# stemangiola/ppcseq

Hardware: AMD Instinct MI355X
Metric: effective samples/sec (whole node) for NB hierarchical fit (higher is better)
Workload: dtype f64; 1 GPU; BASELINE cfg3: synthetic 20000 genes x 200 samples (seed 20253), C=2, K=1000; NUTS (Stan defaults) warm-up 150 + 250 kept draws/chain, 8 chains per GPU (cfg3 names 8 chains; chains are the sharded unit, so N GPUs run 8N chains); mode=chains, chains_total=8, lanes_per_gene=4, loglik_workgroups=939, ess_estimator=rank-normalised split-chain bulk-ESS, min over 6 hyper-parameters and lp__, grad_evals=1471121, divergent_after_warmup=0, round_structure=pipelined: merged log-likelihood / state-machine launch + gene kernel, stream_groups=library default (3 from eight chains on, 2 from four), rounds_last_step_all_groups=115040

## Files before the change

ppcseq_amd/build.py:

```python
from __future__ import annotations

import os
import subprocess
import sys
import threading

HERE = os.path.dirname(os.path.abspath(__file__))
CSRC = os.path.join(HERE, "csrc")
LIB = os.path.join(HERE, "libppcx.so")
TESTING_LIB = os.path.join(os.path.dirname(HERE), "tests", "libppcx_testing.so")
SOURCES = ["ppcx_kernels.hip", "ppcx_summary.hip", "ppcx_psis.hip", "ppcx_loo.hip", "ppcx_loo_predict.hip", "ppcx_reff.hip", "ppcx_ppc_exact.hip", "ppcx_ppc.hip",
           "ppcx_capi.hip", "ppcx_run.hip", "ppcx_fit_nuts.hip", "ppcx_fit_advi.hip", "ppcx_fit_api.hip"]
TESTING_SOURCES = ["ppcx_testing_math.hip"]
HEADERS = ["ppcx_math.h", "ppcx_disp.h", "ppcx_model.h", "ppcx_nuts.h", "ppcx_gene.h", "ppcx_kernels.h", "ppcx_summary.h", "ppcx_summary_dev.h", "ppcx_psis.h", "ppcx_psis_dev.h", "ppcx_loo.h", "ppcx_loo_ap.h", "ppcx_loo_dev.h", "ppcx_loo_predict.h", "ppcx_reff.h", "ppcx_nbcdf.h", "ppcx_ppc_exact.h", "ppcx_ppc.h", "ppcx_table.h", "ppcx_block.h", "ppcx_columns.h", "ppcx_host.h", "ppcx_testing.h",
           os.path.join("..", "..", "include", "ppcx.h")]


CODEGEN_FLAGS = ["-fno-slp-vectorize"]


def _sources(extra):
    return SOURCES + (TESTING_SOURCES if "-DPPCX_TESTING" in extra else [])


def _stale(lib: str, extra=()) -> bool:
    if not os.path.exists(lib):
        return True
    t = os.path.getmtime(lib)
    return any(os.path.getmtime(os.path.join(CSRC, f)) > t for f in _sources(extra) + HEADERS)


_COMPILERS = threading.BoundedSemaphore(16)


def _start_compiler(cmd):
    _COMPILERS.acquire()
    p = subprocess.Popen(cmd)
# ... 65 lines not shown
```

ppcseq_amd/csrc/ppcx_capi.hip:

```cpp
#include <math.h>
#include <stdlib.h>
#include <algorithm>
#include <memory>
#include "ppcx_host.h"

thread_local std::string g_err;
int fail(int code, const std::string& msg) { g_err = msg; return code; }
int hip_fail(hipError_t e, const char* what) { return fail(PPCX_ERR_HIP, std::string(what) + ": " + hipGetErrorString(e)); }
int hip_done(const char* who, hipError_t e) {
  return e == hipSuccess ? PPCX_OK : who ? hip_fail(e, who) : fail(PPCX_ERR_HIP, hipGetErrorString(e));
}
#ifdef PPCX_TESTING
TestHooks g_test;
#endif

extern "C" int ppcx_version(void) { return PPCX_VERSION; }
extern "C" int ppcx_device_count(void) { int n = 0; if (hipGetDeviceCount(&n) != hipSuccess) return 0; return n; }
extern "C" const char* ppcx_last_error(void) { return g_err.c_str(); }
extern "C" int ppcx_device_memory(int device, unsigned long long* free_bytes, unsigned long long* total_bytes) {
  int ndev = 0;
  HIPCHK(hipGetDeviceCount(&ndev));
  if (device < 0 || device >= ndev) return fail(PPCX_ERR_ARG, "no such HIP device");
  HIPCHK(hipSetDevice(device));
  size_t f = 0, t = 0;
  HIPCHK(hipMemGetInfo(&f, &t));
  if (free_bytes) *free_bytes = (unsigned long long)f;
  if (total_bytes) *total_bytes = (unsigned long long)t;
  return PPCX_OK;
}

static double pass_cost(const ppcx_model* m, int L, int p, int n) {
  const int S = m->d.S;
  bool slope = false;
  for (int i = p; i < p + n; ++i) slope = slope || m->pos_slope[i];
  double slope_w = m->d.C > 2 ? 1.0 : 1.15;
#ifdef PPCX_TESTING
  if (g_test.slope_cost_permille > 0) slope_w = 1e-3 * g_test.slope_cost_permille;
#endif
  double lin_w = 2.5;
#ifdef PPCX_TESTING
  if (g_test.slope_cost_permille > 0) lin_w = 1e-3 * g_test.slope_cost_permille;
#endif
  const double sweep = (double)((S + L - 1) / L) * (!m->d.x0_is_one ? 2.5 : (slope && !m->d.x1_binary ? lin_w : (slope ? slope_w : 1.0)));
  return 5.8 + sweep;
}
static int resident_workgroups(const ppcx_model* m, int reserve) {
  int n = m->wgs_override > 0 ? m->wgs_override : m->n_cu * (reserve > 0 ? m->ls_wgs_per_cu : m->wgs_per_cu);
  n -= reserve;
  return n < 1 ? 1 : n;
}
constexpr double kTrimSlack = 0.0;
static int workgroups_per_chain(const ppcx_model* m, int L, int nch, int n_res, bool whole_runs = true, bool trim = false) {
  int nbpc = n_res / (nch < 1 ? 1 : nch);
  if (nbpc >= 8 && whole_runs) nbpc = nbpc / 8 * 8;
  if (nbpc < 1) nbpc = 1;
  const int gpw = 64 / L, npass = (m->d.G + gpw - 1) / gpw;
  if (nbpc > (npass + 3) / 4) nbpc = (npass + 3) / 4;
  if (trim) {
    double slack = kTrimSlack;
#ifdef PPCX_TESTING
    if (g_test.trim_slack_permille >= 0) slack = 1e-3 * g_test.trim_slack_permille;
#endif
    int maxp = (npass + 4 * nbpc - 1) / (4 * nbpc);
#ifdef PPCX_TESTING
    maxp += g_test.trim_extra_passes;
// ... 63 lines not shown
    const long pmax = ((long)(npass + wpc - 1) / wpc) * gpw;
    for (int j = 0; j < wpc; ++j) if (bounds[j + 1] - bounds[j] > pmax) bounds[j + 1] = (int)(bounds[j] + pmax);
    bounds[wpc] = G;
    for (int j = wpc - 1; j >= 0; --j) if (bounds[j + 1] - bounds[j] > pmax) bounds[j] = (int)(bounds[j + 1] - pmax);
  }
  DeviceBuffer<int> d_bounds;
  HIPCHK(d_bounds.alloc((size_t)(wpc + 1)));
  HIPCHK(hipMemcpy(d_bounds.p, bounds.data(), sizeof(int) * (size_t)(wpc + 1), hipMemcpyHostToDevice));
  ppcx_model::Plan& pl = m->plans[key];
  pl.nbpc = nbpc; std::swap(pl.d_bounds.p, d_bounds.p);
  *nbpc_out = pl.nbpc; *d_bounds_out = pl.d_bounds.p;
  return PPCX_OK;
}

static int upload_counts(ppcx_model* m, int n_excl, const int32_t* excl) {
  const int G = m->d.G, S = m->d.S, C = m->d.C;
  std::vector<int32_t> cnt(m->counts_host);
  for (int e = 0; e < n_excl; ++e) {
    if (excl[e] < 0 || excl[e] >= G * S) return fail(PPCX_ERR_ARG, "excluded cell id out of range");
    cnt[excl[e]] = -1;
  }
  std::vector<double> Sy(G, 0.0), SyE(G, 0.0), SyX((size_t)C * G, 0.0), SX((size_t)C * G, 0.0), ncell(G, 0.0), Lg1(G, 0.0);
  std::vector<unsigned char> gflags(G, 0);
  for (int g = 0; g < G; ++g) {
    double sy = 0, sye = 0, nc = 0, lg1 = 0;
    for (int s = 0; s < S; ++s) {
      const int y = cnt[(size_t)g * S + s];
      if (y < 0) { gflags[g] |= 1; continue; }
      sy += y; sye += (double)y * m->expo_host[s]; nc += 1.0; lg1 += lgamma((double)y + 1.0);
      for (int c = 0; c < C; ++c) { SyX[(size_t)c * G + g] += (double)y * m->X_host[(size_t)c * S + s]; SX[(size_t)c * G + g] += m->X_host[(size_t)c * S + s]; }
    }
    Sy[g] = sy; SyE[g] = sye; ncell[g] = nc; Lg1[g] = lg1;
  }
  HIPCHK(hipMemcpy(m->d_gflags.p, gflags.data(), (size_t)G, hipMemcpyHostToDevice));
  {
    std::vector<int> ord(G);
    for (int g = 0; g < G; ++g) ord[g] = g;
    const int K = m->d.K;
    std::stable_sort(ord.begin(), ord.end(), [&](int a, int b) {
      const bool sa = a < K && C >= 2, sb = b < K && C >= 2;
      if (sa != sb) return sa;
      return gflags[a] > gflags[b];
    });
    {
      int ns = 0;
      while (ns < G && ord[ns] < K && C >= 2) ++ns;
      constexpr int kOrderBlock = 16;
      const int nbs = (ns + kOrderBlock - 1) / kOrderBlock, nb = (G + kOrderBlock - 1) / kOrderBlock;
      const bool dear_slopes = m->d.x0_is_one && !m->d.x1_binary;
      if (ns > 0 && ns < G && nbs < nb && dear_slopes) {
        std::vector<int> mixed; mixed.reserve(G);
        int is = 0, ip = ns, sb = 0;
        for (int b = 0; b < nb; ++b) {
          const bool slope_block = sb < nbs && b == (int)((long long)sb * nb / nbs);
          if (slope_block && is < ns) { for (int k = 0; k < kOrderBlock && is < ns; ++k) mixed.push_back(ord[is++]); ++sb; }
          else { for (int k = 0; k < kOrderBlock && ip < G; ++k) mixed.push_back(ord[ip++]); }
        }
        while (is < ns) mixed.push_back(ord[is++]);
        while (ip < G) mixed.push_back(ord[ip++]);
        ord.swap(mixed);
      }
    }
    HIPCHK(hipMemcpy(m->d_order.p, ord.data(), sizeof(int) * (size_t)G, hipMemcpyHostToDevice));
    m->pos_slope.resize(G);
    for (int p = 0; p < G; ++p) m->pos_slope[p] = ord[p] < K && C >= 2;
    drop_plans(m);
  }
  HIPCHK(hipMemcpy(m->d_counts.p, cnt.data(), sizeof(int32_t) * cnt.size(), hipMemcpyHostToDevice));
  m->excluded_host.assign(cnt.size(), 0);
  for (size_t i = 0; i < cnt.size(); ++i) m->excluded_host[i] = cnt[i] < 0;
  {
    const hipError_t e = launch_disp_build_kernel(m->d_counts.p, G, S, nullptr, G, m->fit, m->d_disp.p, m->stream.s);
    if (e != hipSuccess) return fail(PPCX_ERR_HIP, std::string("dispersion-table kernel: ") + hipGetErrorString(e));
  }
  HIPCHK(hipMemcpy(m->d_Sy.p, Sy.data(), sizeof(double) * G, hipMemcpyHostToDevice));
  HIPCHK(hipMemcpy(m->d_SyE.p, SyE.data(), sizeof(double) * G, hipMemcpyHostToDevice));
  HIPCHK(hipMemcpy(m->d_SyX.p, SyX.data(), sizeof(double) * SyX.size(), hipMemcpyHostToDevice));
  HIPCHK(hipMemcpy(m->d_SX.p, SX.data(), sizeof(double) * SX.size(), hipMemcpyHostToDevice));
  HIPCHK(hipMemcpy(m->d_ncell.p, ncell.data(), sizeof(double) * G, hipMemcpyHostToDevice));
  HIPCHK(hipMemcpy(m->d_Lg1.p, Lg1.data(), sizeof(double) * G, hipMemcpyHostToDevice));
  HIPCHK(hipStreamSynchronize(m->stream.s));
  return PPCX_OK;
}

extern "C" int ppcx_model_create(int device, int G, int S, int C, int K, const int32_t* counts, const double* X,
                                 const double* exposure, double lambda_mu_mu, int n_excl, const int32_t* excl,
                                 ppcx_model** out) {
  if (!out) return fail(PPCX_ERR_ARG, "out is NULL");
  *out = nullptr;
  if (G < 1 || S < 1 || C < 1 || K < 0 || K > G) return fail(PPCX_ERR_ARG, "need G>=1, S>=1, C>=1, 0<=K<=G");
  if (C > kMaxC) return fail(PPCX_ERR_LIMIT, "C exceeds the 16 design columns this build supports");
  if ((long long)G * S > 2000000000LL) return fail(PPCX_ERR_LIMIT, "G*S exceeds int32 cell ids");
  if (!counts || !X || !exposure || (n_excl > 0 && !excl)) return fail(PPCX_ERR_ARG, "NULL input buffer");
  for (long long i = 0; i < (long long)G * S; ++i) if (counts[i] < 0) return fail(PPCX_ERR_ARG, "negative count");
  int ndev = 0;
  HIPCHK(hipGetDeviceCount(&ndev));
  if (device < 0 || device >= ndev) return fail(PPCX_ERR_ARG, "no such HIP device");
// ... 25 lines not shown
    return fail(PPCX_ERR_LIMIT, "more than 8 design columns are supported for designs of a column of ones and 0 / 1 indicator columns only");
  if (const char* e = getenv("PPCX_PIPELINE")) if (atoi(e) == 0) m->opt_pipelined = 0;
  if (const char* e = getenv("PPCX_STREAM_GROUPS")) { const int v = atoi(e); if (v >= 1) m->opt_stream_groups = v; }
  if (loglik_lds_bytes(m->d) > 160u * 1024u)
    return fail(PPCX_ERR_LIMIT, "the per-sample constants (S * C doubles; S * (2 + C) for a design without a column of ones) do not fit the 160 KB of LDS of a compute unit beside the 20 KB of tables");
  m->wgs_per_cu = loglik_resident_workgroups_per_cu(m->CM, m->d);
  if (m->wgs_per_cu < 1) return fail(PPCX_ERR_LIMIT, "the log-likelihood kernel cannot be resident with S * (2 + C) doubles of per-sample constants in LDS");
  m->ls_wgs_per_cu = ls_resident_workgroups_per_cu(m->CM, m->d);
  std::vector<double> E(S);
  for (int s = 0; s < S; ++s) E[s] = exp(exposure[s]);
  HIPCHK(m->stream.create());
  HIPCHK(m->d_counts.alloc(((size_t)G * S + 512)));
  HIPCHK(hipMemset(m->d_counts.p, 0, sizeof(int32_t) * ((size_t)G * S + 512)));
  HIPCHK(m->d_E.alloc(S));
  HIPCHK(m->d_expo.alloc(S));
  HIPCHK(m->d_X.alloc((size_t)S * C));
  HIPCHK(m->d_Sy.alloc(G));
  HIPCHK(m->d_SyE.alloc(G));
  HIPCHK(m->d_SyX.alloc((size_t)C * G));
  HIPCHK(m->d_SX.alloc((size_t)C * G));
  HIPCHK(m->d_ncell.alloc(G));
  HIPCHK(m->d_disp.alloc((size_t)G * kDispGeneDoubles));
  HIPCHK(m->d_gflags.alloc((size_t)G));
  disp_fit_init(m->fit);
  HIPCHK(m->d_Lg1.alloc(G));
  HIPCHK(m->d_logtab.alloc(2 * kLogTabSize));
  { double tab[2 * kLogTabSize]; fill_log_table(tab); HIPCHK(hipMemcpy(m->d_logtab.p, tab, sizeof(tab), hipMemcpyHostToDevice)); }
  HIPCHK(m->d_wintab.alloc(2 * kWinTabSize));
  { std::vector<double> wt(2 * kWinTabSize); fill_window_log_table(wt.data()); HIPCHK(hipMemcpy(m->d_wintab.p, wt.data(), sizeof(double) * wt.size(), hipMemcpyHostToDevice)); }
  m->e_min = m->e_max = E[0];
  for (int s = 1; s < S; ++s) { if (E[s] < m->e_min) m->e_min = E[s]; if (E[s] > m->e_max) m->e_max = E[s]; }
  HIPCHK(m->d_order.alloc((size_t)G));
  HIPCHK(hipMemcpy(m->d_E.p, E.data(), sizeof(double) * S, hipMemcpyHostToDevice));
  HIPCHK(hipMemcpy(m->d_expo.p, exposure, sizeof(double) * S, hipMemcpyHostToDevice));
  HIPCHK(hipMemcpy(m->d_X.p, X, sizeof(double) * (size_t)S * C, hipMemcpyHostToDevice));
  const int rc = upload_counts(m, n_excl, excl);
  if (rc != PPCX_OK) return rc;
  choose_launch(m, 1);
  *out = owner.release();
  return PPCX_OK;
}
extern "C" int ppcx_model_create_shard_strided(int device, int G_total, int S, int C, int K_total, int g0, int gene_stride, int n_genes,
                                               const int32_t* counts_shard, const double* X, const double* exposure,
                                               double lambda_mu_mu, int n_excl, const int32_t* excl_local, ppcx_model** out) {
  if (g0 < 0 || gene_stride < 1 || n_genes < 1 || K_total < 0 || K_total > G_total ||
      (long long)g0 + (long long)gene_stride * (n_genes - 1) >= G_total) return fail(PPCX_ERR_ARG, "bad gene shard");
// ... 108 lines not shown
```

ppcseq_amd/csrc/ppcx_gene.h:

```cpp
#pragma once
#include "ppcx_nuts.h"


namespace ppcx {

template <int CM>
struct GeneCtx {
  static constexpr int NCM = CM + 1;
  int gg, ncoord;
  bool active, has_slopes, fast, two;
  int idx[NCM];
  double q[NCM];
  GeneParams<CM> gp;
};

PPCX_HD void coord_consts(const Dims& d, const VecRef& v, int i, double q) {
  if (i >= d.off_sigma_raw && i < d.off_tail) {
    v.at(V_C0, i) = fast_exp(-q); v.at(V_C2, i) = q;
  } else if (i >= d.off_intercept && i < d.off_sigma_raw) {
    v.at(V_C0, i) = fast_exp(q);
    if (d.raw_consts) v.at(V_C2, i) = q;
  }
}

// ... 17 lines not shown
  x.gp.coef[0] = x.q[0];
#pragma unroll
  for (int cc = 1; cc < CM; ++cc) x.gp.coef[cc] = (x.has_slopes && cc < d.C) ? x.q[cc + 1] : 0.0;
  x.gp.sigma_raw = x.q[1];
  x.gp.phi = x.active ? v.at(V_C0, x.idx[1]) : 1.0;
  x.gp.invphi = 0.0;
}
template <int CM>
PPCX_HD void gene_load(const Dims& d, const Cmd& c, const VecRef& v, int g, GeneCtx<CM>& x) {
  constexpr int NCM = CM + 1;
  gene_index<CM>(d, g, x);
#pragma unroll
  for (int j = 0; j < NCM; ++j) x.q[j] = j < x.ncoord ? v.at(V_Q0 + 3 * c.dir, x.idx[j]) : 0.0;
  gene_params<CM>(d, v, x);
}

struct CellData {
  const int* counts;
  const double* disp;
  const unsigned char* gflags;
  const double* Sy;
  const double* ncell;
  double e_min, e_max;
};

struct GenePre { double phi, sigma, a0, Sy, n; int flags; };
PPCX_HD GenePre gene_pre_load(const Dims& d, const VecRef& v, const CellData& m, int g) {
  GenePre r;
  r.phi = v.at(V_C0, d.off_sigma_raw + g);
  r.sigma = v.at(V_C2, d.off_sigma_raw + g);
  r.a0 = v.at(V_C0, d.off_intercept + g);
  r.Sy = m.Sy[g]; r.n = m.ncell[g]; r.flags = m.gflags[g];
  return r;
}
template <int L> struct DispDeal {
  static constexpr int NL = L >= 8 ? 4 : (L >= 4 ? 2 : 1);
  static constexpr int CH = kDispStride / NL;
};

template <int CM, int L, int MODE, bool MASKED, bool WIN>
PPCX_HD void sweep_cells(int S, const int* row, const double* sE, const double* sX1, int sub, double A, double A1, double one,
                         const GeneParams<CM>& gp, const double* tab, CellAcc<CM>& acc, const double* ec = nullptr, int C = 2) {
  const int nmin = S / L;
  const int nlane = nmin + (sub < S - nmin * L ? 1 : 0);
  const int* p = row + sub;
  const double* q = sE + sub;
  const double* qx = sX1 + sub;
  int y0 = p[0], y1 = p[L], y2 = p[2 * L], y3 = p[3 * L];
  int k = 0;
#define PPCX_SWEEP_CELL(Y, E, XB, OFF, COND)                                                    \
  if ((COND) && (!MASKED || (Y) >= 0)) {                                                        \
    if (MODE == 1) { const double a1_ = (XB) != 0.0 ? A1 : A;                                   \
                     const double rho_ = WIN ? cell_eval_win<CM, true>(Y, E, a1_, one, gp, tab, acc) : cell_eval<CM, true>(Y, E, a1_, gp, tab, acc); \
                     acc.Tx[1] = fma(XB, rho_, acc.Tx[1]); }                                    \
    else if (MODE == 2) {                                                                       \
      double a_ = (XB) != 0.0 ? A1 : A; double xk_[CM];                                         \
      _Pragma("unroll") for (int cc = 2; cc < CM; ++cc) { xk_[cc] = cc < C ? qx[(cc - 1) * S + (OFF)] : 0.0; a_ = xk_[cc] != 0.0 ? a_ * ec[cc] : a_; } \
      const double rho_ = WIN ? cell_eval_win<CM, true>(Y, E, a_, one, gp, tab, acc) : cell_eval<CM, true>(Y, E, a_, gp, tab, acc); \
      acc.Tx[1] = fma(XB, rho_, acc.Tx[1]);                                                     \
      _Pragma("unroll") for (int cc = 2; cc < CM; ++cc) acc.Tx[cc] = fma(xk_[cc], rho_, acc.Tx[cc]); \
// ... 100 lines not shown
  const double sigma = pre.sigma;
  gp.sigma_raw = sigma;
  gp.invphi = fast_rcp(gp.phi);
  const double A = pre.a0 * gp.invphi;
  const bool masked = (pre.flags & 1) != 0;
  const int* row = m.counts + (long)g * S;
  constexpr int NL = DispDeal<L>::NL, CH = DispDeal<L>::CH;
  const DispRef dr = disp_ref(sigma);
  const int fn = L == 1 ? 0 : sub / NL, jch = L == 1 ? 0 : sub - fn * NL;
  const bool tab_lane = dr.in && (L == 1 || fn < 2);
  const double* pc = m.disp + (((long)g * kDispPanels + dr.panel) * 2 + (fn & 1)) * kDispStride + jch * CH;
  double cf[CH], cf2[L == 1 ? CH : 1];
#pragma unroll
  for (int k = 0; k < CH; ++k) cf[k] = 0.0;
  cf2[0] = 0.0;
  if (tab_lane) {
#pragma unroll
    for (int k = 0; k < CH; ++k) cf[k] = pc[k];
    if (L == 1) {
#pragma unroll
      for (int k = 0; k < CH; ++k) cf2[k] = pc[kDispStride + k];
    }
  }
  CellAcc<CM> acc; acc.zero();
  PPCX_GSTAMP(5);
  if (GEN & 2) {
    if (PPCX_WAVE_ANY(generic)) {
      if (generic) generic_cells<CM, L>(d, c, v, g, has_slopes, row, sExpo, sX, sub, gp, tab, acc);
    }
  }
  GeneWindow gw; gw.k = 0; gw.ok = false; gw.scale = 1.0;
  bool win = false;
  if (!(GEN & 2) || PPCX_WAVE_ANY(!generic)) {
    if (!generic) {
      const bool any_masked = PPCX_WAVE_ANY(masked);
#define PPCX_SWEEP(MODE, A_LO, A_HI, A_, A1_, X1_, ...)                                                                  \
      gw = gene_window(fma(m.e_min, A_LO, 1.0), fma(m.e_max, A_HI, 1.0));                                                 \
      win = !any_masked && PPCX_WAVE_ALL(gw.ok);                                                                          \
      if (any_masked) sweep_cells<CM, L, MODE, true, false>(S, row, sE, X1_, sub, A_, A1_, 1.0, gp, tab, acc, ##__VA_ARGS__);   \
      else if (win) sweep_cells<CM, L, MODE, false, true>(S, row, sE, X1_, sub, (A_) * gw.scale, (A1_) * gw.scale, gw.scale, gp, wtab, acc, ##__VA_ARGS__); \
      else sweep_cells<CM, L, MODE, false, false>(S, row, sE, X1_, sub, A_, A1_, 1.0, gp, tab, acc, ##__VA_ARGS__);
      if ((GEN & 1) && PPCX_WAVE_ANY(lin)) {
        double be[CM];
        be[0] = 0.0;
#pragma unroll
        for (int cc = 1; cc < CM; ++cc) be[cc] = (lin && cc < d.C) ? v.at(V_C2, coef_index(d, cc, g)) : 0.0;
        if (any_masked) sweep_cells<CM, L, 3, true, false>(S, row, sE, sX + S, sub, A, A, 1.0, gp, tab, acc, be, d.C);
        else sweep_cells<CM, L, 3, false, false>(S, row, sE, sX + S, sub, A, A, 1.0, gp, tab, acc, be, d.C);
      } else if (CM > 2 && d.C > 2 && PPCX_WAVE_ANY(two)) {
        double ec[CM];
        ec[0] = 1.0;
        double a_lo = A, a_hi = A;
#pragma unroll
        for (int cc = 1; cc < CM; ++cc) {
          ec[cc] = (two && cc < d.C) ? v.at(V_C0, coef_index(d, cc, g)) : 1.0;
          a_lo = ec[cc] < 1.0 ? a_lo * ec[cc] : a_lo; a_hi = ec[cc] > 1.0 ? a_hi * ec[cc] : a_hi;
        }
        const double A1 = A * ec[1];
        PPCX_SWEEP(2, a_lo, a_hi, A, A1, sX + S, ec, d.C)
      } else if (PPCX_WAVE_ANY(two)) {
        const double A1 = two ? A * v.at(V_C0, coef_index(d, 1, g)) : A;
        PPCX_SWEEP(1, (A1 < A ? A1 : A), (A1 > A ? A1 : A), A, A1, sX + S)
      } else {
        PPCX_SWEEP(0, A, A, A, A, sX)
      }
#undef PPCX_SWEEP
    }
  }
  PPCX_GSTAMP(6);
  if (!win) gw.scale = 1.0;
  cell_acc_close<CM>(gp, acc, gw.scale, &o);
  if ((GEN & 1) && lin) o.Tx[0] = o.Sr;
  if (win && sub == 0 && gw.k != 0) {
    const double kd = (double)gw.k;
    const double klog2 = fma(kd, 6.93147180369123816490e-01, kd * 1.90821492927058770002e-10);
    o.lik -= klog2 * fma(gp.phi, pre.n, pre.Sy);
    o.dph -= klog2 * pre.n;
  }
  if (tab_lane) {
    double hv = cf[CH - 1];
#pragma unroll
    for (int k = CH - 2; k >= 0; --k) hv = fma(hv, dr.x, cf[k]);
    if (NL > 1) {
      const double x3 = dr.x * dr.x * dr.x, xc = CH == 3 ? x3 : x3 * x3;
      double xp = (jch & 1) ? xc : 1.0;
      if (NL > 2) xp = (jch & 2) ? xp * (xc * xc) : xp;
      hv *= xp;
    }
    if (L == 1) {
      double h2 = cf2[CH - 1];
#pragma unroll
      for (int k = CH - 2; k >= 0; --k) h2 = fma(h2, dr.x, cf2[k]);
      o.lik += hv; o.dph += h2;
    } else if (fn == 0) o.lik += hv;
    else o.dph += hv;
  }
  if (PPCX_WAVE_ANY(!dr.in)) {
    PPCX_KEEP_BRANCH();
    if (!dr.in) {
      double F, D;
      disp_row_at(row, S, sub, L, sigma, &F, &D);
      o.lik += F; o.dph += D;
    }
  }
}

struct GeneData { double Sy, SyE, ncell, Lg1, SyX[kMaxC], SX[kMaxC]; };
template <int CM>
PPCX_HD void gene_data_load(const Dims& d, int gg, const double* Sy, const double* SyE, const double* SyXg, const double* SXg,
                            const double* ncell, const double* Lg1, GeneData& o) {
  o.Sy = Sy[gg]; o.SyE = SyE[gg]; o.ncell = ncell[gg]; o.Lg1 = Lg1[gg];
#pragma unroll
  for (int cc = 0; cc < CM; ++cc) {
    if (cc == 0 && d.x0_is_one) { o.SyX[0] = o.Sy; o.SX[0] = o.ncell; continue; }
    o.SyX[cc] = (cc < d.C) ? SyXg[(long)cc * d.G + gg] : 0.0;
    o.SX[cc] = (cc < d.C) ? SXg[(long)cc * d.G + gg] : 0.0;
  }
}
// ... 221 lines not shown
```

ppcseq_amd/csrc/ppcx_host.h:

```cpp
#pragma once
#include <hip/hip_runtime.h>
#include <atomic>
#include <map>
#include <mutex>
#include <string>
#include <vector>
#include "../../include/ppcx.h"
#include "ppcx_kernels.h"
#include "ppcx_columns.h"

using namespace ppcx;

extern thread_local std::string g_err;
int fail(int code, const std::string& msg);
int hip_fail(hipError_t e, const char* what);
int hip_done(const char* who, hipError_t e);
#define HIPCHK(expr)                                                                       \
  do {                                                                                     \
    hipError_t e_ = (expr);                                                                \
    if (e_ != hipSuccess) return hip_fail(e_, #expr);                                      \
  } while (0)

#ifdef PPCX_TESTING
#include "ppcx_testing.h"
// ... 12 lines not shown
#endif

struct ppcx_model {
  int device;
  DeviceStream stream;
  Dims d;
  int CM, L = 64;
  int L_override = 0, wgs_override = 0;
  int n_cu = 256, wgs_per_cu = 4;
  int ls_wgs_per_cu = 0;
  int nblocks_chosen = 0;
  int opt_pipelined = -1, opt_stream_groups = 0;
  ppcx_progress_fn progress = nullptr; void* progress_user = nullptr; double progress_every = 1.0;
  std::vector<char> pos_slope;
  struct Plan { int nbpc = 0; DeviceBuffer<int> d_bounds; };
  std::map<std::pair<int, int>, Plan> plans;
  std::mutex plan_mutex;
  std::vector<int32_t> counts_host;
  std::vector<char> excluded_host;
  std::vector<double> X_host, expo_host;
  DeviceBuffer<int> d_counts;
  DeviceBuffer<double> d_E, d_expo, d_X, d_Sy, d_SyE, d_SyX, d_SX, d_ncell, d_Lg1;
  DeviceBuffer<double> d_disp;
  DeviceBuffer<unsigned char> d_gflags;
  DispFit fit;
  DeviceBuffer<double> d_logtab, d_wintab;
  double e_min = 1.0, e_max = 1.0;
  DeviceBuffer<int> d_order;
  int live_fits = 0;
  bool destroy_requested = false;
};

struct ppcx_fit {
  ppcx_model* m;
  NutsConfig cfg;
  int chains, n_keep, iter;
  DeviceBuffer<double> d_draws;
  DeviceBuffer<double> d_lp, d_stepsize, d_accept;
  DeviceBuffer<int> d_treedepth, d_nleap, d_div;
  double seconds = 0; long long grad_evals = 0;
  double kA_ms_mean = 0; long long kA_samples = 0; double kA_chain_launches_mean = 0;
  double kC_ms_mean = 0, kU_ms_mean = 0; long long launch_triples = 0;
  double advi_elbo = 0, advi_eta = 0; int advi_converged = 0;
  double ppc_ms = 0; long long ppc_draws = 0;
  long long xchg_ticks = 0, xchg_count = 0;
  std::vector<double> inv_metric;
// ... 46 lines not shown
```

ppcseq_amd/csrc/ppcx_kernels.h:

```cpp
#pragma once
#include <hip/hip_runtime.h>
#include "ppcx_gene.h"

namespace ppcx {

constexpr int kLdsPad = 256;
struct LoglikArgs {
  Dims d;
  CellData cd;
  const double* sampleE;
  const double* exposure;
  const double* X;
  double* vecs;
  long Dpad;
  const Cmd* cmds;
  double* sums;
  const double* logtab;
  const double* wintab;
  const int* order;
  int lgL;
  int nchains;
  const int* active;
  int nbpc;
  const int* bounds;
// ... 92 lines not shown
  const double* exposure; const double* X;
  double truncation_compensation, p_lo, p_hi;
  uint32_t k0;
  int n_gen, resample, n_cells;
  double* ci;
  int* counts_rng;
  int* scratch;
};

hipError_t launch_loglik_kernel(int CM, const LoglikArgs& a, hipStream_t st);
int loglik_resident_workgroups_per_cu(int CM, const Dims& d);
size_t loglik_lds_bytes(const Dims& d);
hipError_t launch_close_kernel(int CM, const CloseArgs& a, int nblocks, int nchains, hipStream_t st);
hipError_t launch_ls_kernel(int CM, const LoglikArgs& a, const StepArgs& sa, int n_srun, int n_chains_total, int spec, hipStream_t st,
                            hipEvent_t ev_start = nullptr, hipEvent_t ev_stop = nullptr);
int ls_resident_workgroups_per_cu(int CM, const Dims& d);
hipError_t launch_gene_kernel(int CM, const GeneArgs& a, int nblocks, int nchains, hipStream_t st);
hipError_t launch_step_kernel(const StepArgs& a, int nblocks, int nchains, hipStream_t st);
hipError_t launch_sum_shards_kernel(const ShardSumArgs& a, hipStream_t st);
hipError_t launch_update_kernel(const UpdateArgs& a, int nblocks, int nchains, hipStream_t st);
hipError_t launch_advi_kernel(const AdviArgs& a, int nblocks, hipStream_t st);
hipError_t launch_advi_elbo_kernel(const AdviElboArgs& a, hipStream_t st);
hipError_t launch_disp_build_kernel(const int* counts, int G, int S, const int* genes, int n_genes, const DispFit& fit, double* table, hipStream_t st);
hipError_t launch_gather_kernel(const double* draws, long n_rows, int D, const int* cols, int n_cols, double* out, hipStream_t st);
hipError_t launch_fill_kernel(double* p, long n, double val, hipStream_t st);

constexpr int kSummaryLdsDraws = 8192;
constexpr int kSummaryMaxChains = 128;
struct SummaryArgs {
  const double* x;
  int n_cols, M, n;
  int npad;
  double* out;
  double* scratch; long slice;
};
int summary_npad(int M, int n);
long summary_slice_doubles(int M, int n);
size_t summary_lds_bytes(int M, int n);
hipError_t launch_summary_gather_kernel(const double* draws, const double* lp, long rows, int D, const int* cols, int n_cols, double* out, hipStream_t st);
hipError_t launch_summary_kernel(const SummaryArgs& a, int nblocks, hipStream_t st);
constexpr size_t kSummaryScratchBytes = (size_t)256 << 20;
hipError_t summary_columns(const double* draws, const double* lp, int M, int n, int D, int n_cols, const int* cols, double* out,
                           size_t scratch_bytes, hipStream_t st);

constexpr int kPsisLdsDraws = 4096;
constexpr int kPsisMaxSel = 4096;
// ... 79 lines not shown
```

ppcseq_amd/csrc/ppcx_kernels.hip:

```cpp
#include <hip/hip_runtime.h>
#include <hip/hip_ext.h>
#include "ppcx_gene.h"
#include "ppcx_kernels.h"

namespace ppcx {

typedef int __attribute__((may_alias)) word_t;
typedef double2 __attribute__((may_alias)) dpair_t;

#ifndef PPCX_LOGLIK_OCC
#define PPCX_LOGLIK_OCC 2
#endif
#ifndef PPCX_LOGLIK_OCC_FAST
#define PPCX_LOGLIK_OCC_FAST 4
#endif
__device__ __forceinline__ double wave_xor_add_rt(double v, int lane_xor_mask) {
  const int src = (int)((threadIdx.x ^ (unsigned)lane_xor_mask) & 63u) << 2;
  const int lo = __builtin_amdgcn_ds_bpermute(src, __double2loint(v));
  const int hi = __builtin_amdgcn_ds_bpermute(src, __double2hiint(v));
  return v + __hiloint2double(hi, lo);
}
template <int CTRL, int ROW_MASK>
__device__ __forceinline__ double dpp_take(double v) {
  const int lo = __builtin_amdgcn_update_dpp(0, __double2loint(v), CTRL, ROW_MASK, 0xf, true);
// ... 884 lines not shown
  double* s_val = reinterpret_cast<double*>(s_row + ((S + 1) & ~1));
  for (int s = tid; s < S; s += kDispThreads) s_row[s] = counts[(long)g * S + s];
  __syncthreads();
  constexpr int NN = kDispPanels * kDispN;
  for (int t = tid; t < NN; t += kDispThreads) {
    const int p = t / kDispN, k = t - p * kDispN;
    double lo;
    const double sg = disp_node_sigma(fit, p, k, &lo);
    const DispPoint pt = disp_point(sg, lo);
    double F, D;
    disp_row(s_row, S, 0, 1, pt, &F, &D);
    s_val[(p * 2 + 0) * kDispN + k] = F; s_val[(p * 2 + 1) * kDispN + k] = D;
  }
  __syncthreads();
  for (int t = tid; t < 2 * kDispPanels; t += kDispThreads) {
    double out[kDispStride];
    disp_fit_panel(fit, s_val + t * kDispN, out);
    double* dst = table + (long)g * kDispGeneDoubles + (long)t * kDispStride;
#pragma unroll
    for (int m = 0; m < kDispStride; ++m) dst[m] = out[m];
  }
}

__global__ void ppcx_gather_kernel(const double* draws, long n_rows, int D, const int* cols, int n_cols, double* out) {
  const long i = (long)blockIdx.x * blockDim.x + threadIdx.x;
  if (i >= n_rows * n_cols) return;
  const long r = i / n_cols; const int cidx = (int)(i % n_cols);
  out[i] = draws[r * D + cols[cidx]];
}

__global__ void ppcx_xchg_abort_kernel(XchgArgs x) {
  const int k = threadIdx.x;
  if (k < x.nranks) sys_store(x.flags[k] + xchg_abort_index(x, x.rank), (unsigned long long)x.epoch);
  __threadfence_system();
}

__global__ void ppcx_fill_kernel(double* p, long n, double val) {
  const long i = (long)blockIdx.x * blockDim.x + threadIdx.x;
  if (i < n) p[i] = val;
}

static int loglik_generic_possible(const Dims& d) { return !d.x0_is_one ? 2 : ((d.C >= 2 && d.K > 0 && !d.x1_binary) ? 1 : 0); }
size_t loglik_lds_bytes(const Dims& d) {
  const size_t per_sample = loglik_generic_possible(d) == 2 ? (size_t)(2 + d.C) : (size_t)(d.C < 1 ? 1 : d.C);
  return sizeof(double) * (2 * kLogTabSize + 2 * kWinTabSize + (size_t)d.S * per_sample + 2 * kLdsPad);
}
// ... 85 lines not shown
}
hipError_t launch_update_kernel(const UpdateArgs& a, int nblocks, int nchains, hipStream_t st) {
  hipLaunchKernelGGL(ppcx_update_kernel, dim3(nblocks, nchains), dim3(256), 0, st, a);
  return hipGetLastError();
}
hipError_t launch_advi_kernel(const AdviArgs& a, int nblocks, hipStream_t st) {
  hipLaunchKernelGGL(ppcx_advi_kernel, dim3(nblocks), dim3(256), 0, st, a);
  return hipGetLastError();
}
hipError_t launch_advi_elbo_kernel(const AdviElboArgs& a, hipStream_t st) {
  hipLaunchKernelGGL(ppcx_advi_elbo_kernel, dim3(1), dim3(64), 0, st, a);
  return hipGetLastError();
}
size_t disp_build_lds_bytes(int S) { return sizeof(int) * (size_t)((S + 1) & ~1) + sizeof(double) * 2 * kDispPanels * kDispN; }
hipError_t launch_disp_build_kernel(const int* counts, int G, int S, const int* genes, int n_genes, const DispFit& fit, double* table, hipStream_t st) {
  const size_t lds = disp_build_lds_bytes(S);
  if (lds > 64u * 1024u) {
    hipError_t e = hipFuncSetAttribute((const void*)ppcx_disp_build_kernel, hipFuncAttributeMaxDynamicSharedMemorySize, (int)lds);
    if (e != hipSuccess) return e;
  }
  hipLaunchKernelGGL(ppcx_disp_build_kernel, dim3((unsigned)n_genes), dim3(kDispThreads), lds, st, counts, G, S, genes, n_genes, fit, table);
  return hipGetLastError();
}
hipError_t launch_gather_kernel(const double* draws, long n_rows, int D, const int* cols, int n_cols, double* out, hipStream_t st) {
  const long n = n_rows * n_cols;
  hipLaunchKernelGGL(ppcx_gather_kernel, dim3((unsigned)((n + 255) / 256)), dim3(256), 0, st, draws, n_rows, D, cols, n_cols, out);
  return hipGetLastError();
}
hipError_t launch_xchg_abort_kernel(const XchgArgs& x, hipStream_t st) {
  hipLaunchKernelGGL(ppcx_xchg_abort_kernel, dim3(1), dim3(64), 0, st, x);
  return hipGetLastError();
}
hipError_t launch_fill_kernel(double* p, long n, double val, hipStream_t st) {
  hipLaunchKernelGGL(ppcx_fill_kernel, dim3((unsigned)((n + 255) / 256)), dim3(256), 0, st, p, n, val);
  return hipGetLastError();
}

}
```

ppcseq_amd/csrc/ppcx_run.hip:

```cpp
#include <stdio.h>
#include <stdlib.h>
#include <string.h>
#include <chrono>
#include <dlfcn.h>
#include "ppcx_host.h"

#ifdef PPCX_TRACE
static unsigned long long* g_trace_dev = nullptr;
#endif
int work_alloc(Work& w, ppcx_model* m, int nchains) {
  const int D = m->d.D;
  if (!w.stream) w.stream = m->stream.s;
  w.Dpad = ((long)D + 31) / 32 * 32;
  w.nb_update = (D + 255) / 256;
  if (w.nb_update > 80) w.nb_update = 80;
  if (w.nb_update < 1) w.nb_update = 1;
  HIPCHK(w.vecs.alloc((size_t)nchains * V_COUNT * w.Dpad));
  w.nb_close = (m->d.G + 255) / 256;
  HIPCHK(w.partials.alloc((size_t)nchains * w.nb_close * PT_COUNT));
  HIPCHK(w.sums.alloc((size_t)nchains * (3 + m->CM) * m->d.G));
  HIPCHK(hipMemsetAsync(w.sums.p, 0, sizeof(double) * (size_t)nchains * (3 + m->CM) * m->d.G, w.stream));
  HIPCHK(w.done.alloc(nchains));
  HIPCHK(w.red.alloc((size_t)nchains * PT_COUNT));
  HIPCHK(hipMemsetAsync(w.red.p, 0, sizeof(double) * (size_t)nchains * PT_COUNT, w.stream));
// ... 43 lines not shown
}
int launch_step(ppcx_model* m, Work& w, int nchains, const RunIO& io, int phases, bool with_update) {
  StepArgs sa;
  step_args(m, w, io, phases, with_update, &sa);
  hipError_t e = launch_step_kernel(sa, w.nb_update, nchains, w.stream);
  if (e != hipSuccess) return fail(PPCX_ERR_HIP, std::string("step kernel: ") + hipGetErrorString(e));
  if (phases & STEP_ADVANCE) w.launches++;
  return PPCX_OK;
}
int launch_update(ppcx_model* m, Work& w, int nchains, const RunIO& io) {
  UpdateArgs ua;
  ua.d = m->d; ua.cmds = w.cmds[w.launches & 1].p; ua.vecs = w.vecs.p; ua.Dpad = w.Dpad;
  ua.draws = io.draws; ua.draws_chain_stride = io.draws_stride; ua.t0_out = w.t0[w.launches & 1].p;
  hipError_t e = launch_update_kernel(ua, w.nb_update, nchains, w.stream);
  if (e != hipSuccess) return fail(PPCX_ERR_HIP, std::string("update kernel: ") + hipGetErrorString(e));
  return PPCX_OK;
}
static int step_runs(int nchains, int nact) { return (nchains + nact - 1) / nact; }
static int loglik_args(ppcx_model* m, Work& w, int nchains, int reserve, LoglikArgs* out) {
  const int nact = w.n_active > 0 ? w.n_active : nchains;
  LoglikArgs& la = *out;
  int rc = plan_launch(m, nact, reserve, w.shared_chip, &la.nbpc, &la.bounds);
  if (rc != PPCX_OK) return rc;
  la.d = m->d; la.cd.counts = m->d_counts.p; la.cd.disp = m->d_disp.p; la.cd.gflags = m->d_gflags.p; la.cd.Sy = m->d_Sy.p; la.cd.ncell = m->d_ncell.p; la.cd.e_min = m->e_min; la.cd.e_max = m->e_max; la.sampleE = m->d_E.p; la.exposure = m->d_expo.p; la.X = m->d_X.p;
  la.vecs = w.vecs.p; la.Dpad = w.Dpad; la.cmds = w.cmds[w.launches & 1].p; la.sums = w.sums.p; la.logtab = m->d_logtab.p; la.wintab = m->d_wintab.p; la.order = m->d_order.p;
  la.lgL = 0; while ((1 << la.lgL) < m->L) ++la.lgL;
  la.nchains = nact; la.active = w.n_active > 0 ? w.active.p : nullptr;
#ifdef PPCX_TRACE
  la.trace = g_trace_dev;
#endif
  return PPCX_OK;
}
int launch_loglik(ppcx_model* m, Work& w, int nchains) {
  LoglikArgs la;
  int rc = loglik_args(m, w, nchains, 0, &la);
  if (rc != PPCX_OK) return rc;
  hipError_t e = launch_loglik_kernel(m->CM, la, w.stream);
  if (e != hipSuccess) return fail(PPCX_ERR_HIP, std::string("loglik kernel: ") + hipGetErrorString(e));
  return PPCX_OK;
}
static void close_args(ppcx_model* m, Work& w, CloseArgs* o) {
  CloseArgs& ca = *o;
  ca.d = m->d; ca.Sy = m->d_Sy.p; ca.SyE = m->d_SyE.p; ca.SyX = m->d_SyX.p; ca.SX = m->d_SX.p; ca.ncell = m->d_ncell.p; ca.Lg1 = m->d_Lg1.p;
  ca.sums = w.sums.p; ca.vecs = w.vecs.p; ca.Dpad = w.Dpad; ca.cmds = w.cmds[w.launches & 1].p; ca.partials = w.partials.p;
}
static int launch_ls(ppcx_model* m, Work& w, int nchains, const RunIO& io, hipEvent_t ev_start = nullptr, hipEvent_t ev_stop = nullptr) {
  const int nact = w.n_active > 0 ? w.n_active : nchains;
// ... 405 lines not shown
```

Baseline: 462.5 ESS/s.

## Replace per-gene sample sweep with precomputed polynomial tables over intercept

Adds per-gene tables of piecewise polynomial fits, built once at model setup, for the sums over samples that the NB log-likelihood needs as functions of the raw intercept. In the gradient kernel, genes without slopes whose intercept falls inside the tabulated panels evaluate a short polynomial instead of sweeping all S samples. Scheduling costs for such passes are lowered to match. The trade-offs are extra device memory for the tables, a setup-time build kernel, and approximation error from the polynomial fit. Genes with slopes or out-of-range intercepts still take the full sweep.

Result: slower. 291.3 ESS/s (-37.0%).

```diff
diff --git a/ppcseq_amd/build.py b/ppcseq_amd/build.py
--- a/ppcseq_amd/build.py
+++ b/ppcseq_amd/build.py
@@ -12,7 +12,7 @@
 SOURCES = ["ppcx_kernels.hip", "ppcx_summary.hip", "ppcx_psis.hip", "ppcx_loo.hip", "ppcx_loo_predict.hip", "ppcx_reff.hip", "ppcx_ppc_exact.hip", "ppcx_ppc.hip",
            "ppcx_capi.hip", "ppcx_run.hip", "ppcx_fit_nuts.hip", "ppcx_fit_advi.hip", "ppcx_fit_api.hip"]
 TESTING_SOURCES = ["ppcx_testing_math.hip"]
-HEADERS = ["ppcx_math.h", "ppcx_disp.h", "ppcx_model.h", "ppcx_nuts.h", "ppcx_gene.h", "ppcx_kernels.h", "ppcx_summary.h", "ppcx_summary_dev.h", "ppcx_psis.h", "ppcx_psis_dev.h", "ppcx_loo.h", "ppcx_loo_ap.h", "ppcx_loo_dev.h", "ppcx_loo_predict.h", "ppcx_reff.h", "ppcx_nbcdf.h", "ppcx_ppc_exact.h", "ppcx_ppc.h", "ppcx_table.h", "ppcx_block.h", "ppcx_columns.h", "ppcx_host.h", "ppcx_testing.h",
+HEADERS = ["ppcx_math.h", "ppcx_disp.h", "ppcx_samp.h", "ppcx_model.h", "ppcx_nuts.h", "ppcx_gene.h", "ppcx_kernels.h", "ppcx_summary.h", "ppcx_summary_dev.h", "ppcx_psis.h", "ppcx_psis_dev.h", "ppcx_loo.h", "ppcx_loo_ap.h", "ppcx_loo_dev.h", "ppcx_loo_predict.h", "ppcx_reff.h", "ppcx_nbcdf.h", "ppcx_ppc_exact.h", "ppcx_ppc.h", "ppcx_table.h", "ppcx_block.h", "ppcx_columns.h", "ppcx_host.h", "ppcx_testing.h",
            os.path.join("..", "..", "include", "ppcx.h")]
 
 
diff --git a/ppcseq_amd/csrc/ppcx_capi.hip b/ppcseq_amd/csrc/ppcx_capi.hip
--- a/ppcseq_amd/csrc/ppcx_capi.hip
+++ b/ppcseq_amd/csrc/ppcx_capi.hip
@@ -29,6 +29,7 @@
   return PPCX_OK;
 }
 
+constexpr double kSampPassCost = 2.0;
 static double pass_cost(const ppcx_model* m, int L, int p, int n) {
   const int S = m->d.S;
   bool slope = false;
@@ -41,6 +42,7 @@
 #ifdef PPCX_TESTING
   if (g_test.slope_cost_permille > 0) lin_w = 1e-3 * g_test.slope_cost_permille;
 #endif
+  if (!slope && m->d_samp.p) return 5.8 + kSampPassCost;
   const double sweep = (double)((S + L - 1) / L) * (!m->d.x0_is_one ? 2.5 : (slope && !m->d.x1_binary ? lin_w : (slope ? slope_w : 1.0)));
   return 5.8 + sweep;
 }
@@ -150,6 +152,7 @@
   }
   std::vector<double> Sy(G, 0.0), SyE(G, 0.0), SyX((size_t)C * G, 0.0), SX((size_t)C * G, 0.0), ncell(G, 0.0), Lg1(G, 0.0);
   std::vector<unsigned char> gflags(G, 0);
+  std::vector<double> samp_org(m->d_samp.p ? G : 0);
   for (int g = 0; g < G; ++g) {
     double sy = 0, sye = 0, nc = 0, lg1 = 0;
     for (int s = 0; s < S; ++s) {
@@ -159,6 +162,11 @@
       for (int c = 0; c < C; ++c) { SyX[(size_t)c * G + g] += (double)y * m->X_host[(size_t)c * S + s]; SX[(size_t)c * G + g] += m->X_host[(size_t)c * S + s]; }
     }
     Sy[g] = sy; SyE[g] = sye; ncell[g] = nc; Lg1[g] = lg1;
+    if (m->d_samp.p) {
+      double se = 0;
+      for (int s = 0; s < S; ++s) if (cnt[(size_t)g * S + s] >= 0) se += exp(m->expo_host[s]);
+      samp_org[g] = samp_origin(sy, se);
+    }
   }
   HIPCHK(hipMemcpy(m->d_gflags.p, gflags.data(), (size_t)G, hipMemcpyHostToDevice));
   {
@@ -201,6 +209,11 @@
     const hipError_t e = launch_disp_build_kernel(m->d_counts.p, G, S, nullptr, G, m->fit, m->d_disp.p, m->stream.s);
     if (e != hipSuccess) return fail(PPCX_ERR_HIP, std::string("dispersion-table kernel: ") + hipGetErrorString(e));
   }
+  if (m->d_samp.p) {
+    HIPCHK(hipMemcpy(m->d_samp_org.p, samp_org.data(), sizeof(double) * G, hipMemcpyHostToDevice));
+    const hipError_t e = launch_samp_build_kernel(m->d_counts.p, m->d_E.p, m->d_samp_org.p, G, S, C >= 2 ? m->d.K : 0, m->fit, m->d_samp.p, m->stream.s);
+    if (e != hipSuccess) return fail(PPCX_ERR_HIP, std::string("sample-table kernel: ") + hipGetErrorString(e));
+  }
   HIPCHK(hipMemcpy(m->d_Sy.p, Sy.data(), sizeof(double) * G, hipMemcpyHostToDevice));
   HIPCHK(hipMemcpy(m->d_SyE.p, SyE.data(), sizeof(double) * G, hipMemcpyHostToDevice));
   HIPCHK(hipMemcpy(m->d_SyX.p, SyX.data(), sizeof(double) * SyX.size(), hipMemcpyHostToDevice));
@@ -272,6 +285,18 @@
   HIPCHK(m->d_ncell.alloc(G));
   HIPCHK(m->d_disp.alloc((size_t)G * kDispGeneDoubles));
   HIPCHK(m->d_gflags.alloc((size_t)G));
+  {
+    bool want = x0 && (C >= 2 ? K : 0) < G;
+    if (const char* e = getenv("PPCX_SAMPLE_TABLES")) if (atoi(e) == 0) want = false;
+    if (want) {
+      if (m->d_samp.alloc((size_t)G * kSampGeneDoubles) != hipSuccess || m->d_samp_org.alloc((size_t)G) != hipSuccess) {
+        (void)hipGetLastError();
+        (void)hipFree(m->d_samp.p); m->d_samp.p = nullptr;
+        (void)hipFree(m->d_samp_org.p); m->d_samp_org.p = nullptr;
+      }
+    }
+    if (m->d_samp.p) m->d.raw_consts = 1;
+  }
   disp_fit_init(m->fit);
   HIPCHK(m->d_Lg1.alloc(G));
   HIPCHK(m->d_logtab.alloc(2 * kLogTabSize));
diff --git a/ppcseq_amd/csrc/ppcx_gene.h b/ppcseq_amd/csrc/ppcx_gene.h
--- a/ppcseq_amd/csrc/ppcx_gene.h
+++ b/ppcseq_amd/csrc/ppcx_gene.h
@@ -1,5 +1,6 @@
 #pragma once
 #include "ppcx_nuts.h"
+#include "ppcx_samp.h"
 
 
 namespace ppcx {
@@ -63,20 +64,28 @@
   const double* Sy;
   const double* ncell;
   double e_min, e_max;
+  const double* samp = nullptr;
+  const double* samp_org = nullptr;
 };
 
-struct GenePre { double phi, sigma, a0, Sy, n; int flags; };
+struct GenePre { double phi, sigma, a0, Sy, n; int flags; double ai = 0.0, org = 0.0; };
 PPCX_HD GenePre gene_pre_load(const Dims& d, const VecRef& v, const CellData& m, int g) {
   GenePre r;
   r.phi = v.at(V_C0, d.off_sigma_raw + g);
   r.sigma = v.at(V_C2, d.off_sigma_raw + g);
   r.a0 = v.at(V_C0, d.off_intercept + g);
   r.Sy = m.Sy[g]; r.n = m.ncell[g]; r.flags = m.gflags[g];
+  if (m.samp) { r.ai = v.at(V_C2, d.off_intercept + g); r.org = m.samp_org[g]; }
   return r;
 }
 template <int L> struct DispDeal {
   static constexpr int NL = L >= 8 ? 4 : (L >= 4 ? 2 : 1);
   static constexpr int CH = kDispStride / NL;
+};
+template <int L> struct SampDeal {
+  static constexpr int NL = L >= 16 ? 4 : (L >= 8 ? 2 : 1);
+  static constexpr int CH = kDispStride / NL;
+  static constexpr int FPL = L >= 4 ? 1 : kSampFn / L;
 };
 
 template <int CM, int L, int MODE, bool MASKED, bool WIN>
@@ -223,6 +232,9 @@
       for (int k = 0; k < CH; ++k) cf2[k] = pc[kDispStride + k];
     }
   }
+  const SampRef sr = samp_ref(pre.ai, sigma, pre.org);
+  const bool use_samp = m.samp != nullptr && !has_slopes && d.x0_is_one && sr.in;
+  const bool any_sweep = PPCX_WAVE_ANY(!use_samp);
   CellAcc<CM> acc; acc.zero();
   PPCX_GSTAMP(5);
   if (GEN & 2) {
@@ -232,13 +244,14 @@
   }
   GeneWindow gw; gw.k = 0; gw.ok = false; gw.scale = 1.0;
   bool win = false;
-  if (!(GEN & 2) || PPCX_WAVE_ANY(!generic)) {
+  if (any_sweep && (!(GEN & 2) || PPCX_WAVE_ANY(!generic))) {
     if (!generic) {
       const bool any_masked = PPCX_WAVE_ANY(masked);
 #define PPCX_SWEEP(MODE, A_LO, A_HI, A_, A1_, X1_, ...)                                                                  \
       gw = gene_window(fma(m.e_min, A_LO, 1.0), fma(m.e_max, A_HI, 1.0));                                                 \
       win = !any_masked && PPCX_WAVE_ALL(gw.ok);                                                                          \
-      if (any_masked) sweep_cells<CM, L, MODE, true, false>(S, row, sE, X1_, sub, A_, A1_, 1.0, gp, tab, acc, ##__VA_ARGS__);   \
+      if (use_samp) { }                                                                                                   \
+      else if (any_masked) sweep_cells<CM, L, MODE, true, false>(S, row, sE, X1_, sub, A_, A1_, 1.0, gp, tab, acc, ##__VA_ARGS__);   \
       else if (win) sweep_cells<CM, L, MODE, false, true>(S, row, sE, X1_, sub, (A_) * gw.scale, (A1_) * gw.scale, gw.scale, gp, wtab, acc, ##__VA_ARGS__); \
       else sweep_cells<CM, L, MODE, false, false>(S, row, sE, X1_, sub, A_, A1_, 1.0, gp, tab, acc, ##__VA_ARGS__);
       if ((GEN & 1) && PPCX_WAVE_ANY(lin)) {
@@ -246,7 +259,8 @@
         be[0] = 0.0;
 #pragma unroll
         for (int cc = 1; cc < CM; ++cc) be[cc] = (lin && cc < d.C) ? v.at(V_C2, coef_index(d, cc, g)) : 0.0;
-        if (any_masked) sweep_cells<CM, L, 3, true, false>(S, row, sE, sX + S, sub, A, A, 1.0, gp, tab, acc, be, d.C);
+        if (use_samp) { }
+        else if (any_masked) sweep_cells<CM, L, 3, true, false>(S, row, sE, sX + S, sub, A, A, 1.0, gp, tab, acc, be, d.C);
         else sweep_cells<CM, L, 3, false, false>(S, row, sE, sX + S, sub, A, A, 1.0, gp, tab, acc, be, d.C);
       } else if (CM > 2 && d.C > 2 && PPCX_WAVE_ANY(two)) {
         double ec[CM];
@@ -272,7 +286,7 @@
   if (!win) gw.scale = 1.0;
   cell_acc_close<CM>(gp, acc, gw.scale, &o);
   if ((GEN & 1) && lin) o.Tx[0] = o.Sr;
-  if (win && sub == 0 && gw.k != 0) {
+  if (win && !use_samp && sub == 0 && gw.k != 0) {
     const double kd = (double)gw.k;
     const double klog2 = fma(kd, 6.93147180369123816490e-01, kd * 1.90821492927058770002e-10);
     o.lik -= klog2 * fma(gp.phi, pre.n, pre.Sy);
@@ -295,6 +309,36 @@
       o.lik += hv; o.dph += h2;
     } else if (fn == 0) o.lik += hv;
     else o.dph += hv;
+  }
+  if (PPCX_WAVE_ANY(use_samp)) {
+    if (use_samp) {
+      constexpr int SNL = SampDeal<L>::NL, SCH = SampDeal<L>::CH, FPL = SampDeal<L>::FPL;
+      const int f0 = L >= 4 ? sub / SNL : sub * FPL, sj = L >= 4 ? sub - f0 * SNL : 0;
+      if (f0 < kSampFn) {
+        const double* ps = m.samp + (((long)g * kSampPanels + sr.panel) * kSampFn + f0) * kDispStride + sj * SCH;
+        double xp = 1.0;
+        if (SNL > 1) {
+          const double x3 = sr.x * sr.x * sr.x, xc = SCH == 3 ? x3 : x3 * x3;
+          xp = (sj & 1) ? xc : 1.0;
+          if (SNL > 2) xp = (sj & 2) ? xp * (xc * xc) : xp;
+        }
+#pragma unroll
+        for (int i = 0; i < FPL; ++i) {
+          double sc[SCH];
+#pragma unroll
+          for (int k = 0; k < SCH; ++k) sc[k] = ps[i * kDispStride + k];
+          double hv = sc[SCH - 1];
+#pragma unroll
+          for (int k = SCH - 2; k >= 0; --k) hv = fma(hv, sr.x, sc[k]);
+          if (SNL > 1) hv *= xp;
+          const int f = f0 + i;
+          if (f == 0) { o.lik = fma(-gp.phi, hv, o.lik); o.dph -= hv; }
+          else if (f == 1) o.lik -= hv;
+          else if (f == 2) o.Sr += hv;
+          else o.Sr = fma(hv, gp.invphi, o.Sr);
+        }
+      }
+    }
   }
   if (PPCX_WAVE_ANY(!dr.in)) {
     PPCX_KEEP_BRANCH();
diff --git a/ppcseq_amd/csrc/ppcx_host.h b/ppcseq_amd/csrc/ppcx_host.h
--- a/ppcseq_amd/csrc/ppcx_host.h
+++ b/ppcseq_amd/csrc/ppcx_host.h
@@ -58,6 +58,7 @@
   DeviceBuffer<int> d_counts;
   DeviceBuffer<double> d_E, d_expo, d_X, d_Sy, d_SyE, d_SyX, d_SX, d_ncell, d_Lg1;
   DeviceBuffer<double> d_disp;
+  DeviceBuffer<double> d_samp, d_samp_org;
   DeviceBuffer<unsigned char> d_gflags;
   DispFit fit;
   DeviceBuffer<double> d_logtab, d_wintab;
diff --git a/ppcseq_amd/csrc/ppcx_kernels.h b/ppcseq_amd/csrc/ppcx_kernels.h
--- a/ppcseq_amd/csrc/ppcx_kernels.h
+++ b/ppcseq_amd/csrc/ppcx_kernels.h
@@ -138,6 +138,7 @@
 hipError_t launch_advi_kernel(const AdviArgs& a, int nblocks, hipStream_t st);
 hipError_t launch_advi_elbo_kernel(const AdviElboArgs& a, hipStream_t st);
 hipError_t launch_disp_build_kernel(const int* counts, int G, int S, const int* genes, int n_genes, const DispFit& fit, double* table, hipStream_t st);
+hipError_t launch_samp_build_kernel(const int* counts, const double* E, const double* org, int G, int S, int g_begin, const DispFit& fit, double* table, hipStream_t st);
 hipError_t launch_gather_kernel(const double* draws, long n_rows, int D, const int* cols, int n_cols, double* out, hipStream_t st);
 hipError_t launch_fill_kernel(double* p, long n, double val, hipStream_t st);
 
diff --git a/ppcseq_amd/csrc/ppcx_kernels.hip b/ppcseq_amd/csrc/ppcx_kernels.hip
--- a/ppcseq_amd/csrc/ppcx_kernels.hip
+++ b/ppcseq_amd/csrc/ppcx_kernels.hip
@@ -930,6 +930,36 @@
   }
 }
 
+__global__ __launch_bounds__(kDispThreads) void ppcx_samp_build_kernel(const int* counts, const double* E, const double* org, int G, int S,
+                                                                        int g_begin, DispFit fit, double* table) {
+  extern __shared__ int s_row[];
+  const int g = g_begin + blockIdx.x;
+  if (g >= G) return;
+  const int tid = threadIdx.x;
+  double* s_E = reinterpret_cast<double*>(s_row + ((S + 1) & ~1));
+  double* s_val = s_E + S;
+  for (int s = tid; s < S; s += kDispThreads) { s_row[s] = counts[(long)g * S + s]; s_E[s] = E[s]; }
+  __syncthreads();
+  const double o = org[g];
+  constexpr int NN = kSampPanels * kDispN;
+  for (int t = tid; t < NN; t += kDispThreads) {
+    const int p = t / kDispN, k = t - p * kDispN;
+    double lo, v4[kSampFn];
+    const double an = samp_node(fit, o, p, k, &lo);
+    samp_row(s_row, s_E, S, 0, 1, samp_node_A(an, lo), v4);
+#pragma unroll
+    for (int fn = 0; fn < kSampFn; ++fn) s_val[(p * kSampFn + fn) * kDispN + k] = v4[fn];
+  }
+  __syncthreads();
+  for (int t = tid; t < kSampFn * kSampPanels; t += kDispThreads) {
+    double out[kDispStride];
+    disp_fit_panel(fit, s_val + t * kDispN, out);
+    double* dst = table + (long)g * kSampGeneDoubles + (long)t * kDispStride;
+#pragma unroll
+    for (int m = 0; m < kDispStride; ++m) dst[m] = out[m];
+  }
+}
+
 __global__ void ppcx_gather_kernel(const double* draws, long n_rows, int D, const int* cols, int n_cols, double* out) {
   const long i = (long)blockIdx.x * blockDim.x + threadIdx.x;
   if (i >= n_rows * n_cols) return;
@@ -1061,6 +1091,16 @@
   hipLaunchKernelGGL(ppcx_disp_build_kernel, dim3((unsigned)n_genes), dim3(kDispThreads), lds, st, counts, G, S, genes, n_genes, fit, table);
   return hipGetLastError();
 }
+hipError_t launch_samp_build_kernel(const int* counts, const double* E, const double* org, int G, int S, int g_begin, const DispFit& fit, double* table, hipStream_t st) {
+  if (g_begin >= G) return hipSuccess;
+  const size_t lds = sizeof(int) * (size_t)((S + 1) & ~1) + sizeof(double) * ((size_t)S + (size_t)kSampFn * kSampPanels * kDispN);
+  if (lds > 64u * 1024u) {
+    hipError_t e = hipFuncSetAttribute((const void*)ppcx_samp_build_kernel, hipFuncAttributeMaxDynamicSharedMemorySize, (int)lds);
+    if (e != hipSuccess) return e;
+  }
+  hipLaunchKernelGGL(ppcx_samp_build_kernel, dim3((unsigned)(G - g_begin)), dim3(kDispThreads), lds, st, counts, E, org, G, S, g_begin, fit, table);
+  return hipGetLastError();
+}
 hipError_t launch_gather_kernel(const double* draws, long n_rows, int D, const int* cols, int n_cols, double* out, hipStream_t st) {
   const long n = n_rows * n_cols;
   hipLaunchKernelGGL(ppcx_gather_kernel, dim3((unsigned)((n + 255) / 256)), dim3(256), 0, st, draws, n_rows, D, cols, n_cols, out);
diff --git a/ppcseq_amd/csrc/ppcx_run.hip b/ppcseq_amd/csrc/ppcx_run.hip
--- a/ppcseq_amd/csrc/ppcx_run.hip
+++ b/ppcseq_amd/csrc/ppcx_run.hip
@@ -89,7 +89,7 @@
   LoglikArgs& la = *out;
   int rc = plan_launch(m, nact, reserve, w.shared_chip, &la.nbpc, &la.bounds);
   if (rc != PPCX_OK) return rc;
-  la.d = m->d; la.cd.counts = m->d_counts.p; la.cd.disp = m->d_disp.p; la.cd.gflags = m->d_gflags.p; la.cd.Sy = m->d_Sy.p; la.cd.ncell = m->d_ncell.p; la.cd.e_min = m->e_min; la.cd.e_max = m->e_max; la.sampleE = m->d_E.p; la.exposure = m->d_expo.p; la.X = m->d_X.p;
+  la.d = m->d; la.cd.counts = m->d_counts.p; la.cd.disp = m->d_disp.p; la.cd.gflags = m->d_gflags.p; la.cd.Sy = m->d_Sy.p; la.cd.ncell = m->d_ncell.p; la.cd.e_min = m->e_min; la.cd.e_max = m->e_max; la.cd.samp = m->d_samp.p; la.cd.samp_org = m->d_samp_org.p; la.sampleE = m->d_E.p; la.exposure = m->d_expo.p; la.X = m->d_X.p;
   la.vecs = w.vecs.p; la.Dpad = w.Dpad; la.cmds = w.cmds[w.launches & 1].p; la.sums = w.sums.p; la.logtab = m->d_logtab.p; la.wintab = m->d_wintab.p; la.order = m->d_order.p;
   la.lgL = 0; while ((1 << la.lgL) < m->L) ++la.lgL;
   la.nchains = nact; la.active = w.n_active > 0 ? w.active.p : nullptr;
diff --git a/ppcseq_amd/csrc/ppcx_samp.h b/ppcseq_amd/csrc/ppcx_samp.h
--- /dev/null
+++ b/ppcseq_amd/csrc/ppcx_samp.h
@@ -0,0 +1,63 @@
+#pragma once
+#include "ppcx_disp.h"
+
+namespace ppcx {
+
+constexpr int kSampPanels = 32, kSampFn = 4;
+constexpr long kSampGeneDoubles = (long)kSampPanels * kSampFn * kDispStride;
+
+inline double samp_origin(double sum_y, double sum_E) {
+  double c = sum_E > 0.0 ? log((sum_y + 0.5) / sum_E) - 2.0 : 0.0;
+  if (!(c > -40.0)) c = -40.0;
+  if (!(c < 40.0)) c = 40.0;
+  const double span = kSampPanels * kDispWidth;
+  const double lo = c <= -0.5 ? c - 4.0 : (c + 4.0 - span > -4.5 ? c + 4.0 - span : -4.5);
+  return floor(lo * kDispInvWidth) * kDispWidth;
+}
+
+PPCX_HD void samp_row(const int* row, const double* E, int S, int start, int stride, double A, double* out) {
+  DispSum sl, sa, sq, syq;
+  for (int s = start; s < S; s += stride) {
+    const int y = row[s];
+    if (y < 0) continue;
+    const double yd = (double)y, z = E[s] * A;
+    const double l = log1p_acc(z), q = 1.0 / (1.0 + z);
+    sl.add(l); sa.add(yd * l); sq.add(q); syq.add(yd * q);
+  }
+  out[0] = sl.value(); out[1] = sa.value(); out[2] = sq.value(); out[3] = syq.value();
+}
+PPCX_HD double samp_node(const DispFit& f, double org, int panel, int k, double* lo) {
+  return disp_node_sigma(f, panel + (int)((org - kDispLo) * kDispInvWidth), k, lo);
+}
+PPCX_HD double samp_node_A(double a, double lo) {
+  const double Ah = fast_exp(a);
+  return fma(lo, Ah, Ah);
+}
+inline void samp_build_gene_host(const DispFit& f, const int* row, const double* E, int S, double org, double* out ) {
+  for (int p = 0; p < kSampPanels; ++p) {
+    double fv[kSampFn][kDispN];
+    for (int k = 0; k < kDispN; ++k) {
+      double lo, v4[kSampFn];
+      const double a = samp_node(f, org, p, k, &lo);
+      samp_row(row, E, S, 0, 1, samp_node_A(a, lo), v4);
+      for (int fn = 0; fn < kSampFn; ++fn) fv[fn][k] = v4[fn];
+    }
+    for (int fn = 0; fn < kSampFn; ++fn) disp_fit_panel(f, fv[fn], out + ((long)p * kSampFn + fn) * kDispStride);
+  }
+}
+
+struct SampRef { int panel; bool in; double x; };
+PPCX_HD SampRef samp_ref(double ai, double sg, double org) {
+  SampRef r;
+  const double a = ai + sg, bb = a - ai;
+  const double err = (ai - (a - bb)) + (sg - bb);
+  const double t = (a - org) * kDispInvWidth;
+  r.in = t >= 0.0 && t < (double)kSampPanels;
+  const int pi = r.in ? (int)t : 0;
+  r.panel = pi;
+  r.x = fma(a - fma((double)pi, kDispWidth, org), 2.0 * kDispInvWidth, -1.0);
+  r.x = fma(err, 2.0 * kDispInvWidth, r.x);
+  return r;
+}
+
+}
```
